# 2lambda123/CliMA-Oceananigans.jl

Hardware: AMD Instinct MI355X
Metric: cell-updates/sec per time_step!, 256^3 Nonhydrostatic WENO5 (higher is better)
Workload: dtype f64

## Files before the change

### clima-oceananigans.jl_amd/csrc/api.hip

```cpp
#include <cstdarg>

#include "internal.h"

#ifdef OCN_HOST_EMU
thread_local dim3 threadIdx, blockIdx, blockDim, gridDim;
emu_barrier g_emu_barrier;
double g_emu_shfl[4096];
std::recursive_mutex g_emu_launch_mutex;
#else
thread_local int g_ocn_dry = 0;
thread_local ocn_launch_error g_ocn_launch_err = {hipSuccess, {0}};
#endif
thread_local int g_ocn_capturing = 0, g_ocn_capture_poison = 0;

static char g_last_error[512] = {0};
static int pnhs_refresh(ocn_model* m);

void ocn_set_error(ocn_ctx* ctx, const char* fmt, ...) {
  va_list ap;
  va_start(ap, fmt);
  vsnprintf(g_last_error, sizeof(g_last_error), fmt, ap);
  va_end(ap);
  if (ctx) memcpy(ctx->err, g_last_error, sizeof(g_last_error));
}
// ... 493 lines not shown
static int pnhs_refresh(ocn_model* m) {
  if (!m->pnhs_halo_stale) return OCN_OK;
  if (int rc = halo_settle(m)) return rc;
  m->pnhs_halo_stale = false;
  Field* fs[1] = {&m->pNHS};
  return comm_halo_exchange_z(m, fs, 1);
}
static int halo_settle_others(ocn_model* m) {
  for (ocn_model* o : m->ctx->models)
    if (o != m)
      if (int rc = halo_settle_one(o)) return rc;
  return OCN_OK;
}

static int overlap_streams(ocn_ctx* c) {
  if (c->overlap_ready) return OCN_OK;
  OCN_HIP_CHECK(c, hipStreamCreate(&c->comm_stream));
  OCN_HIP_CHECK(c, hipEventCreate(&c->ev_main));
  OCN_HIP_CHECK(c, hipEventCreate(&c->ev_halo));
  OCN_HIP_CHECK(c, hipEventCreate(&c->ev_halo2));
  c->overlap_ready = true;
  return OCN_OK;
}

static int fused_substep(ocn_model* m, double dt_full, double cn, double cm, int use_m, double dt_stage, bool swap) {
  const int Hz = m->gd.Hz, Nz = m->gd.Nz;
  if (m->g->dist)
    if (int rc0 = halo_settle_others(m)) return rc0;
  if (m->halo_inflight && Nz > 2 * Hz + 2) {
    launch_fused_tend_step(m, dt_full, cn, cm, use_m, Hz, Nz - Hz);
    OCN_HIP_CHECK(m->ctx, hipStreamWaitEvent(m->ctx->stream, m->ctx->ev_halo, 0));
    m->halo_inflight = false;
    launch_fused_tend_step(m, dt_full, cn, cm, use_m, 0, Hz, Nz - Hz, Nz);
  } else {
    int rc0 = halo_settle(m);
    if (rc0) return rc0;
    launch_fused_tend_step(m, dt_full, cn, cm, use_m);
  }
  launch_tracer_steps(m, dt_full, cn, cm, use_m);
  if (m->halo2_inflight) {
    OCN_HIP_CHECK(m->ctx, hipStreamWaitEvent(m->ctx->stream, m->ctx->ev_halo2, 0));
    m->halo2_inflight = false;
  }
  int rc = OCN_OK;
  if (m->g->dist && !poisson_local_wstar(m) && (rc = fused_exchange_ws(m))) return rc;
  if (poisson_custom_xy(m)) {
    rc = poisson_run_from_predictor(m, dt_stage);
  } else {
    launch_rhs_wrap(m, dt_stage, poisson_rhs_buffer(m->solver));
    rc = poisson_run(m);
  }
  if (rc) return rc;
  if (m->g->dist && !poisson_local_phi_below(m) && (rc = fused_exchange_phi(m, poisson_rhs_buffer(m->solver)))) return rc;
  launch_project(m, dt_stage, poisson_rhs_buffer(m->solver));
  if (m->g->dist) {
    ocn_ctx* c = m->ctx;
    const size_t halo_bytes = (size_t)(3 + m->nt) * Hz * m->u.sz * sizeof(double);
    const bool want = m->knob_overlap >= 0 ? m->knob_overlap != 0 : (c->nranks > 1 && halo_bytes >= ((size_t)8 << 20));
    if (want && comm_can_overlap(c) && Nz > 2 * Hz + 2 && overlap_streams(c) == OCN_OK) {
      Field* fa[3 + OCN_MAX_TRACERS] = {&m->u, &m->v, &m->w};
      int na = 3;
      for (int t = 0; t < m->nt; ++t) fa[na++] = &m->tr[t];
      OCN_HIP_CHECK(c, hipEventRecord(c->ev_main, c->stream));
      OCN_HIP_CHECK(c, hipStreamWaitEvent(c->comm_stream, c->ev_main, 0));
      if ((rc = comm_halo_exchange_z(m, fa, na, c->comm_stream))) return rc;
      OCN_HIP_CHECK(c, hipEventRecord(c->ev_halo, c->comm_stream));
      m->halo_inflight = true;
    } else {
      Field* fs[3 + OCN_MAX_TRACERS] = {&m->u, &m->v, &m->w};
      int nf = 3;
      for (int t = 0; t < m->nt; ++t) fs[nf++] = &m->tr[t];
      if ((rc = comm_halo_exchange_z(m, fs, nf))) return rc;
    }
    m->pnhs_halo_stale = true;
  }
  if (swap)
    for (int f = 0; f < 3 + m->nt; ++f) std::swap(m->Gn[f], m->Gm[f]);
  return OCN_OK;
}

static void tendencies_and_step(ocn_model* m, double dt, double cn, double cm, int use_m) {
  if (!m->bz_fast) {
    launch_tendencies(m);
    launch_step(m, dt, cn, cm, use_m);
    return;
  }
  const bool tr3 = m->nt > 0 && fused_tracer3_ok(m);
  launch_tendencies(m, true, tr3);
  launch_fused_bz(m, dt, cn, cm, use_m);
  if (tr3) launch_tracer3(m, dt, cn, cm, use_m, true);
  else launch_step(m, dt, cn, cm, use_m, true);
  m->pred_active = true;
}

static int time_step_ab2(ocn_model* m, double dt, int force_euler) {
  bool euler = force_euler || (dt != m->previous_dt);
  double chi = euler ? -0.5 : m->d.chi;
  int rc0 = euler ? zero_Gm(m) : OCN_OK;
  if (rc0) return rc0;
  m->previous_dt = dt;
  if (m->iteration == 0 && (rc0 = update_state(m))) return rc0;
  if (m->fast_path) {
    m->gn_alias_gm = false;
    int rc = fused_substep(m, dt, 1.5 + chi, -(0.5 + chi), 1, dt, true);
    if (rc) return rc;
    m->gn_alias_gm = true;
    m->time += dt;
// ... 724 lines not shown
```

### clima-oceananigans.jl_amd/csrc/compat.h

```cpp
#pragma once

#include <cmath>
#include <cstddef>
#include <cstdint>
#include <cstdio>
#include <cstdlib>
#include <cstring>

#ifndef OCN_HOST_EMU
#include <hip/hip_runtime.h>
#include <hipfft/hipfft.h>

#define OCN_DEVFN __device__ __forceinline__

extern thread_local int g_ocn_dry;

struct ocn_launch_error {
  hipError_t err;
  char what[200];
};
extern thread_local ocn_launch_error g_ocn_launch_err;
static inline void ocn_note_error(hipError_t e, const char* what) {
  if (e == hipSuccess || g_ocn_launch_err.err != hipSuccess) return;
  g_ocn_launch_err.err = e;
  snprintf(g_ocn_launch_err.what, sizeof g_ocn_launch_err.what, "%s", what);
}
template <class K, class... A>
static inline void ocn_launch_impl(const char* what, K kern, dim3 grid, dim3 block, hipStream_t s, A... args) {
  if (g_ocn_dry) return;
  hipLaunchKernelGGL(kern, grid, block, 0, s, args...);
  ocn_note_error(hipGetLastError(), what);
}
#define ocn_launch(...) ocn_launch_impl(#__VA_ARGS__, __VA_ARGS__)
#define ocn_launch_sync(...) ocn_launch_impl(#__VA_ARGS__, __VA_ARGS__)
#define OCN_ASYNC(call) ocn_note_error((call), #call)
#define OCN_SHARED __shared__
#define OCN_SCHED_FENCE() __builtin_amdgcn_sched_barrier(0)
#define OCN_TOUCH3(a, b, c) asm volatile("" ::"v"(a), "v"(b), "v"(c))

typedef __attribute__((address_space(3))) void ocn_lds_void;
typedef const __attribute__((address_space(1))) void ocn_glb_void;
__device__ __forceinline__ void ocn_glds16(const void* src_lane, void* dst_wave_base, int ) {
  __builtin_amdgcn_global_load_lds((ocn_glb_void*)src_lane, (ocn_lds_void*)dst_wave_base, 16, 0, 0);
}
__device__ __forceinline__ double ocn_shfl_next(double x) {
  union { double d; int i[2]; } a, b;
  a.d = x;
  b.i[0] = __builtin_amdgcn_update_dpp(0, a.i[0], 0x130, 0xf, 0xf, false);
  b.i[1] = __builtin_amdgcn_update_dpp(0, a.i[1], 0x130, 0xf, 0xf, false);
  return b.d;
}
__device__ __forceinline__ double ocn_shfl_xor16(double x) {
  union { double d; int i[2]; } a, b;
  a.d = x;
  const int lane = __builtin_amdgcn_mbcnt_hi(~0u, __builtin_amdgcn_mbcnt_lo(~0u, 0u));
  const int addr = (lane ^ 16) << 2;
  b.i[0] = __builtin_amdgcn_ds_bpermute(addr, a.i[0]);
  b.i[1] = __builtin_amdgcn_ds_bpermute(addr, a.i[1]);
  return b.d;
}
#define OCN_WAVE 64
#define OCN_UNIFORM(x) __builtin_amdgcn_readfirstlane(x)

#else
#include <chrono>
#include <condition_variable>
#include <mutex>
#include <thread>
#include <vector>

struct dim3 {
  unsigned x, y, z;
  dim3(unsigned a = 1, unsigned b = 1, unsigned c = 1) : x(a), y(b), z(c) {}
};
extern thread_local dim3 threadIdx, blockIdx, blockDim, gridDim;
#define g_ocn_dry 0
extern std::recursive_mutex g_emu_launch_mutex;

#define __global__
#define __device__
#define __host__
#define __forceinline__ inline
#define __launch_bounds__(...)
#define OCN_DEVFN inline
#define OCN_SHARED static
#define OCN_SCHED_FENCE() ((void)0)
#define OCN_ASYNC(call) ((void)(call))
#define OCN_TOUCH3(a, b, c) ((void)0)

typedef int hipError_t;
enum { hipSuccess = 0, hipErrorOutOfMemory = 2 };
typedef struct emu_stream* hipStream_t;
struct emu_event { std::chrono::steady_clock::time_point t; };
typedef emu_event* hipEvent_t;
enum { hipMemcpyHostToDevice = 1, hipMemcpyDeviceToHost = 2, hipMemcpyDeviceToDevice = 3 };

static inline const char* hipGetErrorString(hipError_t) { return "host-emu error"; }
static inline hipError_t hipSetDevice(int) { return 0; }
static inline hipError_t hipGetDeviceCount(int* n) { *n = 1; return 0; }
static inline hipError_t hipStreamCreate(hipStream_t* s) { *s = nullptr; return 0; }
static inline hipError_t hipStreamDestroy(hipStream_t) { return 0; }
static inline hipError_t hipStreamSynchronize(hipStream_t) { return 0; }
static inline hipError_t hipDeviceSynchronize() { return 0; }
static inline hipError_t hipGetLastError() { return 0; }
static inline hipError_t hipMalloc(void** p, size_t n) { *p = malloc(n ? n : 1); return *p ? 0 : 2; }
static inline hipError_t hipFree(void* p) { free(p); return 0; }
static inline hipError_t hipMemcpy(void* d, const void* s, size_t n, int) { memcpy(d, s, n); return 0; }
static inline hipError_t hipMemcpyAsync(void* d, const void* s, size_t n, int, hipStream_t) { memmove(d, s, n); return 0; }
static inline hipError_t hipMemsetAsync(void* d, int v, size_t n, hipStream_t) { memset(d, v, n); return 0; }
static inline hipError_t hipMemset(void* d, int v, size_t n) { memset(d, v, n); return 0; }
static inline hipError_t hipEventCreate(hipEvent_t* e) { *e = new emu_event; return 0; }
static inline hipError_t hipEventDestroy(hipEvent_t e) { delete e; return 0; }
static inline hipError_t hipEventRecord(hipEvent_t e, hipStream_t) { e->t = std::chrono::steady_clock::now(); return 0; }
static inline hipError_t hipEventSynchronize(hipEvent_t) { return 0; }
static inline hipError_t hipStreamWaitEvent(hipStream_t, hipEvent_t, unsigned) { return 0; }
static inline hipError_t hipEventElapsedTime(float* ms, hipEvent_t a, hipEvent_t b) {
  *ms = std::chrono::duration<float, std::milli>(b->t - a->t).count();
  return 0;
}

template <class K, class... A>
static inline void ocn_launch(K kern, dim3 grid, dim3 block, hipStream_t, A... args) {
  std::lock_guard<std::recursive_mutex> lk(g_emu_launch_mutex);
  gridDim = grid;
  blockDim = block;
  for (unsigned bz = 0; bz < grid.z; ++bz)
    for (unsigned by = 0; by < grid.y; ++by)
      for (unsigned bx = 0; bx < grid.x; ++bx) {
        blockIdx = dim3(bx, by, bz);
        for (unsigned tz = 0; tz < block.z; ++tz)
          for (unsigned ty = 0; ty < block.y; ++ty)
            for (unsigned tx = 0; tx < block.x; ++tx) {
              threadIdx = dim3(tx, ty, tz);
              kern(args...);
            }
      }
}

struct emu_barrier {
  std::mutex m;
  std::condition_variable cv;
// ... 70 lines not shown
```

### clima-oceananigans.jl_amd/csrc/fused.hip

```cpp
#include "internal.h"

#define FUSED_MAX_THREADS 1024

struct FusedArgs {
  const double *u, *v, *w;
  const double *gmu, *gmv, *gmw;
  double *gnu, *gnv, *gnw;
  double *us, *vs, *ws;
  unsigned org;
  double dt, cn, cm;
  int use_m;
  int BYo;
  int ntiles;
  int ntx, BXo;
  int prio;
  double nu;
  int zlo, zhi;
  int zlo2, zhi2;
  int gran;
};

#ifndef OCN_HOST_EMU
#define OCN_SETPRIO(n) __builtin_amdgcn_s_setprio(n)
#else
// ... 469 lines not shown
          fxn[0 * BY * NW] = t11;
          fxn[1 * BY * NW] = t12;
          fxn[2 * BY * NW] = t13;
        }
      }
      if (full) {
        if (k > k0) {
          const unsigned cm1 = c - szb;
          const double rzc = ZB ? g_rdzc(g, k - 1) : g.rdz, rzfm = ZB ? g_rdzf(g, k - 1) : g.rdz;
          sto(a.gu, cm1, hu + 2.0 * ((t13 - bu) * rzc));
          sto(a.gv, cm1, hv + 2.0 * ((t23 - bv) * rzc));
          sto(a.gw, cm1, hw + 2.0 * ((t33 - bw) * rzfm));
        }
        if (!last) {
          double cu = 0, cv = 0;
          if (a.coriolis) {
            cu = a.f * (0.5 * (0.5 * (RS(1, 0, -1) + vc) + 0.5 * (RS(1, 1, -1) + RS(1, 1, 0))));
            cv = -a.f * (0.5 * (0.5 * (RS(0, -1, 0) + RS(0, -1, 1)) + 0.5 * (uc + RS(0, 0, 1))));
          }
          if (a.pH) {
            cu -= (p0 - pw) * rdx;
            cv -= (p0 - ps) * rdy;
          }
          hu = cu + 2.0 * fma(xedge ? -t11 : e0 - t11, rdx, -t12 * rdy);
          hv = cv + 2.0 * fma(xedge ? -t12 : e1 - t12, rdx, -t22 * rdy);
          hw = 2.0 * fma(xedge ? -t13 : e2 - t13, rdx, -t23 * rdy);
          bu = t13;
          bv = t23;
          bw = t33;
        }
      }
      up = uc; vp = vc; wp = wc;
      ncp = nc; nwp = nw; nsp = ns;
    }
  }
#undef RS
}

__global__ void k_rhs_wrap(GridDev g, const double* __restrict__ us, const double* __restrict__ vs,
                           const double* __restrict__ ws, double rdt, int zwrap, double* __restrict__ rhs) {
  int i, j;
  ocn_cell_ij(i, j);
  const int k = blockIdx.z;
  if (i >= g.Nx || j >= g.Ny || k >= g.Nz) return;
  const long sy = g.sy, sz = g.sz;
  const long c = i + j * sy + k * sz;
  const long ce = (i + 1 == g.Nx) ? c + 1 - g.Nx : c + 1;
  const long cn = (j + 1 == g.Ny) ? c + sy - g.Ny * sy : c + sy;
  const long ct = (zwrap && k + 1 == g.Nz) ? c + sz - g.Nz * sz : c + sz;
  double div = (us[ce] - us[c]) * g.rdx + (vs[cn] - vs[c]) * g.rdy + (ws[ct] - ws[c]) / g.dz;
  rhs[i + (long)g.Nx * (j + (long)g.Ny * k)] = div * rdt;
}

struct ProjArgs {
  const double* phi;
  const double *us, *vs, *ws;
  double *u, *v, *w, *p;
  const double* phi_below;
  double dt;
  int zwrap;
};

OCN_DEVFN void store_images(const GridDev& g, double* f, int i, int j, int k, double val, int zwrap) {
  long ox[3], oy[3], oz[3];
  int nx = 0, ny = 0, nz = 0;
  ox[nx++] = 0;
  if (i < g.Hx) ox[nx++] = g.Nx;
  if (i >= g.Nx - g.Hx) ox[nx++] = -g.Nx;
  oy[ny++] = 0;
  if (j < g.Hy) oy[ny++] = (long)g.Ny * g.sy;
  if (j >= g.Ny - g.Hy) oy[ny++] = -(long)g.Ny * g.sy;
  oz[nz++] = 0;
  if (zwrap) {
    if (k < g.Hz) oz[nz++] = (long)g.Nz * g.sz;
    if (k >= g.Nz - g.Hz) oz[nz++] = -(long)g.Nz * g.sz;
  }
  const long c = i + j * g.sy + k * g.sz;
  for (int c3 = 0; c3 < nz; ++c3)
    for (int c2 = 0; c2 < ny; ++c2)
      for (int c1 = 0; c1 < nx; ++c1) f[c + ox[c1] + oy[c2] + oz[c3]] = val;
}

__global__ void k_project(GridDev g, ProjArgs a) {
  int i, j;
  ocn_cell_ij(i, j);
  const int k = blockIdx.z;
  if (i >= g.Nx || j >= g.Ny || k >= g.Nz) return;
  const long c = i + j * g.sy + k * g.sz;
  const long Nx = g.Nx, Ny = g.Ny;
  const long pc = i + Nx * (j + Ny * k);
  const long pw_ = (i == 0) ? pc + Nx - 1 : pc - 1;
  const long ps_ = (j == 0) ? pc + Nx * (Ny - 1) : pc - Nx;
  double p0 = a.phi[pc];
  double pb;
  if (k > 0) pb = a.phi[pc - Nx * Ny];
  else if (a.zwrap) pb = a.phi[pc + Nx * Ny * (g.Nz - 1)];
  else pb = a.phi_below[i + Nx * j];
  double un = a.us[c] - (p0 - a.phi[pw_]) * g.rdx * a.dt;
  double vn = a.vs[c] - (p0 - a.phi[ps_]) * g.rdy * a.dt;
  double wn = a.ws[c] - (p0 - pb) / g.dz * a.dt;
  store_images(g, a.u, i, j, k, un, a.zwrap);
  store_images(g, a.v, i, j, k, vn, a.zwrap);
  store_images(g, a.w, i, j, k, wn, a.zwrap);
  store_images(g, a.p, i, j, k, p0, a.zwrap);
}

struct TracerArgs {
  const double *u, *v, *w, *c, *gm;
  double *gn, *cnew;
  double dt, cn, cm;
  int use_m, KZ, zwrap;
  double kappa;
};

template <int ADV>
__global__ void __launch_bounds__(256) k_tracer_step(GridDev g, TracerArgs a) {
  const int i = blockIdx.x * blockDim.x + threadIdx.x;
  const int j = blockIdx.y * blockDim.y + threadIdx.y;
  if (i >= g.Nx || j >= g.Ny) return;
  const int k0 = blockIdx.z * a.KZ;
  const int k1 = (k0 + a.KZ < g.Nz) ? k0 + a.KZ : g.Nz;
  const long sy = g.sy, sz = g.sz;
  const double rdx = g.rdx, rdy = g.rdy, rdz = 1.0 / g.dz;
  long c = i + j * sy + (long)k0 * sz;
  double zc[6];
#pragma unroll
  for (int q = 0; q < 6; ++q) zc[q] = a.c[c + (q - 3) * sz];
  auto fz = [&](long p) {
    const double wt = a.w[p];
    const bool pos = wt > 0.0;
    return wt * recon5<ADV>(pos ? zc[0] : zc[5], pos ? zc[1] : zc[4], pos ? zc[2] : zc[3], pos ? zc[3] : zc[2],
                            pos ? zc[4] : zc[1], pos) - a.kappa * (zc[3] - zc[2]) * rdz;
  };
  double fb = fz(c);
  for (int k = k0; k < k1; ++k, c += sz) {
// ... 171 lines not shown
          const unsigned cm1 = c - szb;
          const double rzc = ZB ? g_rdzc(g, k - 1) : g.rdz;
          const double G = rest - (own_h + (fb - own_b) * rzc);
          sto(a.gn, cm1, G);
          const double inc = a.use_m ? a.dt * (a.cn * G + a.cm * gmv) : a.dt * a.cn * G;
          const double val = zc[2] + inc;
          if (IMG) store_images(g, (double*)((char*)a.cnew + a.org), i, j, k - 1, val, a.zwrap);
          else sto(a.cnew, cm1, val);
        }
        if (!last) {
          own_h = (fxx[nid_e] - fxx[tid]) * rdx + (fxy[nid_n] - fxy[tid]) * rdy;
          own_b = fb;
        }
      }
      if (!last) {
#pragma unroll
        for (int q = 0; q < 5; ++q) zc[q] = zc[q + 1];
        zc[5] = ldo(a.c, c + 3 * szb);
      }
    }
  }
#undef CS
#undef KS
}

static const char* tiled_blocker(const ocn_model* m) {
  const ocn_grid* g = m->g;
  const int adv = m->d.advection;
  if (adv != ADV_WENO_Z && adv != ADV_WENO_JS && adv != ADV_U5) return "the advection scheme is not an upwind-biased 5th-order one";
  for (int d = 0; d < 3; ++d)
    if (g->topo[d] != OCN_FLAT && (g->H[d] < 3 || g->N[d] < 2 * g->H[d])) return "a direction has fewer than 6 cells";
  if (m->u.n * sizeof(double) >= (1ull << 31) || m->w.n * sizeof(double) >= (1ull << 31))
    return "parent arrays of 2 GiB or more exceed the tiled kernels' 32-bit byte offsets";
  return nullptr;
}

bool fused_available(const ocn_model* m) {
  const ocn_grid* g = m->g;
  if (g->topo[0] != OCN_PERIODIC || g->topo[1] != OCN_PERIODIC || g->topo[2] != OCN_PERIODIC) return false;
  if (!g->z_regular) return false;
  if (m->d.closure == OCN_CLOSURE_AMD || m->d.coriolis_fplane || m->d.buoyancy != OCN_BUOYANCY_NONE) return false;
  if (tiled_blocker(m)) return false;
  if (getenv("OCNHIP_NO_FUSED")) return false;
  return true;
}

bool rest4_ok(const ocn_model* m);
void fused_describe(const ocn_model* m, char* buf, size_t n) {
  const char* why = tiled_blocker(m);
  if (m->fast_path) {
    const size_t halo_bytes = (size_t)(3 + m->nt) * m->gd.Hz * m->u.sz * sizeof(double);
    const bool ov = m->g->dist && m->gd.Nz > 2 * m->gd.Hz + 2 &&
                    (m->knob_overlap >= 0 ? m->knob_overlap != 0 : (m->ctx->nranks > 1 && halo_bytes >= ((size_t)8 << 20)));
    snprintf(buf, n, "all-in-one periodic path: k_tend4 + fused Poisson passes + k_project%s",
             !m->g->dist ? "" : ov ? "; z-slabs, halo planes travel under the next interior tendency launch"
                                   : "; z-slabs, halo exchange on the model's stream");
  }
  else if (m->bz_fast) snprintf(buf, n, "tiled advection + update (k_tend4, REST) on top of the %s other terms",
                                rest4_ok(m) ? "tiled kernel's (k_rest4)" : "general kernels'");
  else if (why) snprintf(buf, n, "general kernels: %s", why);
  else if (m->g->topo[0] == OCN_FLAT || m->g->topo[1] == OCN_FLAT) snprintf(buf, n, "general kernels: Flat x / y slices are outside the tiled kernels");
  else snprintf(buf, n, "general kernels (tiled path disabled or not applicable to this topology / decomposition)");
}

static int fused_cu_count(const ocn_model* m) {
  static int ncu = 0;
  if (!ncu) {
#ifndef OCN_HOST_EMU
    hipDeviceProp_t prop;
    ncu = (hipGetDeviceProperties(&prop, m->ctx->device) == hipSuccess) ? prop.multiProcessorCount : 256;
#else
    ncu = 8;
#endif
  }
  return ncu;
}

struct FusedShape {
  int bx, by;
  bool wide, small;
  int dma;
  dim3 blk, grd;
};

void fused_read_knobs(ocn_model* m) {
  auto env = [](const char* n, int def) { const char* e = getenv(n); return e ? atoi(e) : def; };
  m->knob_fused_xt = env("OCNHIP_FUSED_XT", 0);
  m->knob_no_dma = env("OCNHIP_NO_LDS_DMA", 0);
  m->knob_no_tracer3 = env("OCNHIP_NO_TRACER3", 0);
  m->knob_xfft_team = env("OCNHIP_XFFT_TEAM", 0);
  m->knob_overlap = env("OCNHIP_OVERLAP", -1);
  m->knob_overlap_cus = env("OCNHIP_OVERLAP_CUS", 16);
  m->knob_graph = env("OCNHIP_NO_GRAPH", 0) ? 0 : 1;
  { const char* e = getenv("OCNHIP_PRIO"); m->knob_prio = e ? (int)strtol(e, nullptr, 0) : 0x20FF; }
}

static FusedShape fused_shape(const ocn_model* m, FusedArgs& a) {
  const GridDev& gd = m->gd;
  FusedShape f;
  f.small = m->knob_fused_xt == 1 && gd.Nx <= 57 * 4;
#ifdef OCN_HOST_EMU
  if (gd.xb && gd.Nx <= 57 * 4) f.small = true;
#endif
  f.wide = gd.Nx > 256 || f.small || gd.xb;
  f.bx = f.small ? 64 : f.wide ? 192 : gd.Nx <= 64 ? 64 : gd.Nx <= 128 ? 128 : 256;
  f.by = f.small ? 4 : f.wide ? 5 : f.bx == 256 ? 4 : 8;
#ifdef OCN_HOST_EMU
  if ((f.small && gd.Nx <= 36) || (!f.wide && gd.Nx <= 16)) {
    f.bx = 16;
    f.by = 4;
  }
#endif
  a.BYo = f.by - 1;
  a.ntiles = (gd.Ny + f.by - 2) / (f.by - 1);
  a.ntx = 1;
  a.BXo = 0;
  if (f.wide) {
    const int cap = (f.bx - 7) & ~1;
    a.ntx = (gd.Nx + cap - 1) / cap;
    if (f.small && a.ntx < 2) a.ntx = 2;
    a.BXo = (gd.Nx + a.ntx - 1) / a.ntx;
    a.BXo += a.BXo & 1;
    a.ntx = (gd.Nx + a.BXo - 1) / a.BXo;
    a.ntiles *= a.ntx;
  }
  int nseg = fused_cu_count(m);
  const long total = (long)a.ntiles * ((a.zhi - a.zlo) + (a.zhi2 - a.zlo2));
  a.gran = 1;
  if (a.zhi2 > a.zlo2) {
    a.gran = a.zhi - a.zlo;
    const long runs = total / a.gran;
    if (nseg > runs) nseg = (int)runs;
  } else {
    if (a.zhi - a.zlo < gd.Nz && nseg > 4 * m->knob_overlap_cus) nseg -= m->knob_overlap_cus;
    if (nseg > total / 4) nseg = (int)(total / 4 > 8 ? total / 4 : 8);
    nseg = ((nseg + 7) / 8) * 8;
  }
#ifdef OCN_HOST_EMU
  nseg = total >= 3 ? 3 : 1;
#endif
  f.blk = dim3(f.bx, f.by, 1);
  f.grd = dim3(nseg, 1, 1);
  f.dma = (m->knob_no_dma != 1 && gd.Hx == 3 && gd.Nx % 2 == 0 && gd.sy % 2 == 0 && gd.sz % 2 == 0) ? 1 : 0;
// ... 281 lines not shown
```

### clima-oceananigans.jl_amd/csrc/internal.h

```cpp
#pragma once
#include <map>
#include <string>
#include <vector>

#include "../../include/ocnhip.h"
#include "compat.h"
#include "stencils.h"

#define OCN_NF (3 + OCN_MAX_TRACERS)

struct ProfPhase {
  std::vector<std::pair<hipEvent_t, hipEvent_t>> ev;
  double total_ms = 0;
  int64_t count = 0;
};

struct ocn_ctx {
  int device = 0;
  hipStream_t stream = nullptr;
  char err[512] = {0};
  bool profiling = false;
  std::map<std::string, ProfPhase> prof;
  std::string prof_only;
  int rank = 0, nranks = 1;
// ... 41 lines not shown
};

struct Field {
  double* d = nullptr;
  int T[3] = {0, 0, 0};
  int P[3] = {0, 0, 0};
  int off[3] = {0, 0, 0};
  int loc[3] = {0, 0, 0};
  size_t n = 0;
  BCdev bc[6];
  bool present = false;
  double* interior() const;
  long sy = 0, sz = 0;
  int Hx = 0, Hy = 0, Hz = 0;
};

struct PoissonSolver;

struct ocn_model {
  ocn_grid* g;
  ocn_ctx* ctx;
  ocn_model_desc d;
  GridDev gd;
  int nt;
  Field u, v, w, pHY, pNHS;
  Field tr[OCN_MAX_TRACERS], Gn[OCN_NF], Gm[OCN_NF];
  Field nu_e, kappa_e[OCN_MAX_TRACERS];
  Field us, vs, ws;
  Field trs[OCN_MAX_TRACERS];
  PoissonSolver* solver = nullptr;
  std::vector<double*> owned;
  double time = 0, previous_dt = INFINITY;
  int64_t iteration = 0;
  int stage = 1;
  double* d_red = nullptr;
  int fast_path = 0;
  int bz_fast = 0;
  double* amd_tab = nullptr;
  double* phi_below = nullptr;
  double *ypack_s = nullptr, *ypack_r = nullptr;
  size_t ypack_n = 0;
  bool gn_alias_gm = false;
  bool pred_active = false;
  ocn_grid* own_grid = nullptr;
  int knob_fused_xt = 0, knob_no_dma = 0, knob_no_tracer3 = 0, knob_prio = 0x20FF;
  struct StepGraph { uint64_t key; int seen; void* exec; std::vector<uint64_t> words; };
  std::vector<StepGraph> graphs;
  int knob_overlap_cus = 16;
  int knob_overlap = -1;
  bool halo_inflight = false, halo2_inflight = false;
  bool pnhs_halo_stale = false;
  int knob_xfft_team = 0;
  int knob_graph = 1;
  bool graph_off = false;
  int64_t graph_replays = 0;
};
extern thread_local int g_ocn_capturing, g_ocn_capture_poison;
inline Field& pred_u(ocn_model* m) { return m->pred_active ? m->us : m->u; }
inline Field& pred_v(ocn_model* m) { return m->pred_active ? m->vs : m->v; }
inline Field& pred_w(ocn_model* m) { return m->pred_active ? m->ws : m->w; }

Field* model_field(ocn_model* m, int id);

struct FieldPtrs {
  double* p[OCN_NF + 2];
  int Tx[OCN_NF + 2], Ty[OCN_NF + 2], Tz[OCN_NF + 2];
  int n;
};
void launch_fill_periodic(ocn_model* m, const FieldPtrs& f, int dim);
void launch_fill_flat(ocn_model* m, const FieldPtrs& f, int dim);
bool launch_fill_periodic_xy(ocn_model* m, const FieldPtrs& f);
void launch_fill_bounded(ocn_model* m, Field** fs, int n, int dim);
void launch_tendencies(ocn_model* m, bool skip_momentum_advection = false, bool skip_tracer_advection = false);
void launch_step(ocn_model* m, double dt, double cn, double cm, int use_m, bool tracers_only = false);
void launch_store(ocn_model* m);
void launch_rhs(ocn_model* m, double dt, double* rhs, int mult_dz);
void launch_pcorrect(ocn_model* m, double dt);
void launch_hydrostatic(ocn_model* m);
void launch_copy_to_field(ocn_model* m, const double* src, Field& f);
void launch_maxdiv(ocn_model* m, double* out_dev);
void launch_amd(ocn_model* m);
int amd_build_table(ocn_model* m);

void fused_read_knobs(ocn_model* m);
void fused_describe(const ocn_model* m, char* buf, size_t n);
bool fused_available(const ocn_model* m);
bool fused_bz_available(const ocn_model* m);
void launch_fused_bz(ocn_model* m, double dt, double cn, double cm, int use_m);
bool launch_rest4(ocn_model* m);
bool fused_tracer3_ok(const ocn_model* m);
bool tracer_rest_shell(const ocn_model* m);
void launch_tracer3(ocn_model* m, double dt, double cn, double cm, int use_m, bool rest);
void launch_fused_tend_step(ocn_model* m, double dt, double cn, double cm, int use_m, int zlo = 0, int zhi = -1, int zlo2 = 0, int zhi2 = 0);
void launch_rhs_wrap(ocn_model* m, double dt, double* rhs);
void launch_project(ocn_model* m, double dt, const double* phi);
void launch_tracer_steps(ocn_model* m, double dt, double cn, double cm, int use_m);
int fused_exchange_ws(ocn_model* m);
int fused_exchange_phi(ocn_model* m, const double* phi);
int poisson_run(ocn_model* m);

PoissonSolver* poisson_create(ocn_model* m);
void poisson_destroy(PoissonSolver* s);
int poisson_solve(ocn_model* m, double dt);
int poisson_solve_rhs(ocn_model* m, const double* rhs_dev, double* phi_dev);
double* poisson_rhs_buffer(PoissonSolver* s);

void* zsolve_create(ocn_ctx* ctx, const std::vector<double>& lx_half, const std::vector<double>& ly_local);
void zsolve_destroy(void* z);
void zsolve_run(ocn_ctx* ctx, void* z, void* spec, int Nz, const double* lz, double norm, long zero_col);
void yfft_run(ocn_ctx* ctx, void* z, void* spec, int Nxh, int Ny, int Nz, int inverse);
void xfft_rhs_run(ocn_model* m, void* z, void* spec, double dt, int extra_plane = 0);
bool poisson_local_wstar(const ocn_model* m);
bool fft_size_ok(int n);
bool zsolve_size_ok(int n);
bool poisson_custom_xy(const ocn_model* m);
int poisson_run_from_predictor(ocn_model* m, double dt);

void* zslab_create(ocn_ctx* ctx, const std::vector<double>& lx_half, const std::vector<double>& ly, int n, int R, int rank);
void zslab_destroy(void* z);
int zslab_run(ocn_ctx* ctx, void* z, void* spec, double dz2, double scale, const void* below = nullptr, void* phi_below = nullptr);
bool poisson_local_phi_below(const ocn_model* m);
const double* poisson_phi_below(const ocn_model* m);

int comm_exchange(ocn_ctx* c, const std::vector<CommOp>& sends, const std::vector<CommOp>& recvs, hipStream_t st = nullptr);
int comm_halo_exchange_z(ocn_model* m, Field** fs, int n, hipStream_t st = nullptr);
bool comm_can_overlap(const ocn_ctx* c);
int halo_settle(ocn_model* m);
int comm_halo_exchange_y(ocn_model* m, Field** fs, int n);
int comm_alltoall(ocn_ctx* c, const void* send, void* recv, size_t block_bytes);
void comm_destroy(ocn_ctx* c);

struct ProfScope {
  ocn_ctx* c;
  hipEvent_t a = nullptr, b = nullptr;
  const char* name;
  ProfScope(ocn_ctx* ctx, const char* nm);
  ~ProfScope();
};
```

### clima-oceananigans.jl_amd/csrc/poisson.hip

```cpp
#include "internal.h"
#ifndef OCN_HOST_EMU
#define dry_hipfftExecD2Z(...) (g_ocn_dry ? HIPFFT_SUCCESS : hipfftExecD2Z(__VA_ARGS__))
#define dry_hipfftExecZ2D(...) (g_ocn_dry ? HIPFFT_SUCCESS : hipfftExecZ2D(__VA_ARGS__))
#define dry_hipfftExecZ2Z(...) (g_ocn_dry ? HIPFFT_SUCCESS : hipfftExecZ2Z(__VA_ARGS__))
#endif


#ifndef OCN_HOST_EMU
#include <rocblas/rocblas.h>
#endif
#include <complex>
typedef std::complex<double> cplx;

struct double2_ {
  double x, y;
};

struct PoissonSolver {
  int kind;
  int Nx, Ny, Nz, Nxh;
  int R = 1, rank = 0, Nzg = 0, Nyl = 0;
  double2_ *ta = nullptr, *tb = nullptr;
  void* zs = nullptr;
  void* zsl = nullptr;
// ... 1009 lines not shown
  }
  return OCN_OK;
}

int poisson_run(ocn_model* m) { return run_solver(m); }

bool poisson_custom_xy(const ocn_model* m) { return m->solver && m->solver->cxy; }
bool poisson_local_wstar(const ocn_model* m) { return m->solver && m->solver->bplane != nullptr; }
bool poisson_local_phi_below(const ocn_model* m) { return m->solver && m->solver->bplane != nullptr && m->solver->local_phi; }
const double* poisson_phi_below(const ocn_model* m) { return m->solver->rhs + (size_t)m->solver->Nx * m->solver->Ny * m->solver->Nz; }

#ifdef OCN_HOST_EMU
static void emu_xinv(PoissonSolver* s, const double2_* spec = nullptr, double* out = nullptr, size_t nlines = 0) {
  const int Nx = s->Nx, Nxh = s->Nxh;
  const size_t lines = nlines ? nlines : (size_t)s->Ny * s->Nz;
  if (!spec) spec = s->spec;
  if (!out) out = s->rhs;
  std::vector<cplx> full(Nx);
  for (size_t L = 0; L < lines; ++L) {
    for (int i = 0; i < Nx; ++i) {
      double2_ q = spec[(i < Nxh ? i : Nx - i) + Nxh * L];
      full[i] = cplx(q.x, i < Nxh ? q.y : -q.y);
    }
    for (int n = 0; n < Nx; ++n) {
      cplx acc = 0;
      for (int i = 0; i < Nx; ++i) {
        double ang = 2.0 * M_PI * ((long)i * n % Nx) / Nx;
        acc += full[i] * cplx(cos(ang), sin(ang));
      }
      out[n + Nx * L] = acc.real();
    }
  }
}
#endif

int poisson_run_from_predictor(ocn_model* m, double dt) {
  PoissonSolver* s = m->solver;
  const int xp = s->bplane ? 1 : 0, ip = (s->bplane && s->local_phi) ? 1 : 0;
  {
    ProfScope ps(m->ctx, "fft_forward");
    xfft_rhs_run(m, s->tw, s->spec, dt, xp);
    yfft_run(m->ctx, s->tw, s->spec, s->Nxh, s->Ny, s->Nz + xp, 0);
  }
  if (s->zs) {
    ProfScope ps(m->ctx, "spectral_solve");
    zsolve_run(m->ctx, s->zs, s->spec, s->Nz, s->lz, 1.0 / ((double)s->Nx * s->Ny * s->Nz), 0);
  } else {
    int rc = zslab_run(m->ctx, s->zsl, s->spec, s->dz2, 1.0 / ((double)s->Nx * s->Ny), s->bplane, ip ? s->bplane : nullptr);
    if (rc) return rc;
  }
  {
    ProfScope ps(m->ctx, "fft_backward");
    yfft_run(m->ctx, s->tw, s->spec, s->Nxh, s->Ny, s->Nz + ip, 1);
#ifndef OCN_HOST_EMU
    if (dry_hipfftExecZ2D(s->xinv, (hipfftDoubleComplex*)s->spec, s->rhs) != HIPFFT_SUCCESS) {
      ocn_set_error(m->ctx, "hipfftExecZ2D (x inverse) failed");
      return OCN_EHIP;
    }
#else
    emu_xinv(s, s->spec, s->rhs, (size_t)s->Ny * (s->Nz + ip));
#endif
  }
  return OCN_OK;
}

static int poisson_run_from_predictor_bz(ocn_model* m, double dt) {
  PoissonSolver* s = m->solver;
  {
    ProfScope ps(m->ctx, "fft_forward");
    xfft_rhs_run(m, s->tw, s->spec, dt);
    yfft_run(m->ctx, s->tw, s->spec, s->Nxh, s->Ny, s->Nz, 0);
  }
  {
    ProfScope ps(m->ctx, "spectral_solve");
    tridiag_run(m, s, s->Nxh, s->Ny, s->lx, s->ly, 1.0 / ((double)s->Nx * s->Ny), s->spec, 1);
  }
  {
    ProfScope ps(m->ctx, "fft_backward");
    yfft_run(m->ctx, s->tw, s->spec, s->Nxh, s->Ny, s->Nz, 1);
#ifndef OCN_HOST_EMU
    if (dry_hipfftExecZ2D(s->xinv, (hipfftDoubleComplex*)s->spec, s->rhs) != HIPFFT_SUCCESS) {
      ocn_set_error(m->ctx, "hipfftExecZ2D (x inverse) failed");
      return OCN_EHIP;
    }
#else
    emu_xinv(s);
#endif
  }
  return OCN_OK;
}

int poisson_solve(ocn_model* m, double dt) {
  PoissonSolver* s = m->solver;
  int rc;
  if (s->cxy_bz) rc = poisson_run_from_predictor_bz(m, dt);
  else {
    launch_rhs(m, dt, s->rhs, m->g->topo[2] == OCN_BOUNDED ? 1 : 0);
    rc = run_solver(m);
  }
  if (rc) return rc;
  ProfScope ps(m->ctx, "copy_pressure");
  launch_copy_to_field(m, s->rhs, m->pNHS);
  return OCN_OK;
}

__global__ void k_mult_dz(GridDev g, double* __restrict__ r) {
  int i, j;
  ocn_cell_ij(i, j);
  const int k = blockIdx.z;
  if (i >= g.Nx || j >= g.Ny || k >= g.Nz) return;
  r[i + (size_t)g.Nx * (j + (size_t)g.Ny * k)] *= g_dzc(g, k);
}

int poisson_solve_rhs(ocn_model* m, const double* rhs_dev, double* phi_dev) {
  PoissonSolver* s = m->solver;
  size_t nr = (size_t)s->Nx * s->Ny * s->Nz;
  OCN_ASYNC(hipMemcpyAsync(s->rhs, rhs_dev, nr * sizeof(double), hipMemcpyDeviceToDevice, m->ctx->stream));
// ... 10 lines not shown
```

### clima-oceananigans.jl_amd/csrc/zfft.hip

```cpp
#include "internal.h"

struct cd {
  double x, y;
};
OCN_DEVFN cd cadd(cd a, cd b) { return {a.x + b.x, a.y + b.y}; }
OCN_DEVFN cd csub(cd a, cd b) { return {a.x - b.x, a.y - b.y}; }
OCN_DEVFN cd cmul(cd a, cd b) { return {a.x * b.x - a.y * b.y, a.x * b.y + a.y * b.x}; }
template <int S> OCN_DEVFN cd mul_mi(cd a) { return S > 0 ? cd{a.y, -a.x} : cd{-a.y, a.x}; }

template <int S> OCN_DEVFN void dft4(cd& a, cd& b, cd& c, cd& d) {
  cd s0 = cadd(a, c), s1 = csub(a, c), s2 = cadd(b, d), s3 = mul_mi<S>(csub(b, d));
  a = cadd(s0, s2);
  c = csub(s0, s2);
  b = cadd(s1, s3);
  d = csub(s1, s3);
}

template <int S> OCN_DEVFN void dft16(cd* v) {
#pragma unroll
  for (int a = 0; a < 4; ++a) dft4<S>(v[a], v[a + 4], v[a + 8], v[a + 12]);
  const double C1 = 0.92387953251128673848, S1 = 0.38268343236508978178, R = 0.70710678118654752440;
  auto tw = [&](cd z, double c, double s) { return cd{z.x * c + S * z.y * s, z.y * c - S * z.x * s}; };
  v[1 + 4] = tw(v[1 + 4], C1, S1);
  v[1 + 8] = tw(v[1 + 8], R, R);
// ... 428 lines not shown
      const int l2 = e / N, i = e - l2 * N;
      int j = j0 + l2, k = k0;
      while (j >= g.Ny) { j -= g.Ny; ++k; }
      double d = 0.0;
      if (extra && k == g.Nz) d = ws[j * sy + i] * rdz * rdt;
      else if (k < g.Nz) {
        const long row = j * sy + k * sz;
        const long rown = ((j + 1 == g.Ny) ? 0 : j + 1) * sy + k * sz;
        const long rowt = (zwrap && k + 1 == g.Nz) ? j * sy : j * sy + (k + 1) * sz;
        const int ie = (i + 1 == g.Nx) ? 0 : i + 1;
        if (g.zb) {
          const double dzc = g_dzc(g, k);
          d = ((us[row + ie] - us[row + i]) * g.rdx + (vs[rown + i] - vs[row + i]) * g.rdy + (ws[rowt + i] - ws[row + i]) / dzc) * rdt * dzc;
        } else
        d = ((us[row + ie] - us[row + i]) * g.rdx + (vs[rown + i] - vs[row + i]) * g.rdy + (ws[rowt + i] - ws[row + i]) * rdz) * rdt;
      }
      sm[l2 * LP + i] = d;
    }
    __syncthreads();
#pragma unroll
    for (int n1 = 0; n1 < 16; ++n1) v[n1] = {sm[ln * LP + pos_in<N>(r, c, n1)], 0.0};
    __syncthreads();
  } else {
    const int k = ok ? (int)(L / g.Ny) : 0, j = ok ? (int)(L - (long)k * g.Ny) : 0;
    const long row = j * sy + k * sz;
    const long rown = ((j + 1 == g.Ny) ? 0 : j + 1) * sy + k * sz;
    const long rowt = (zwrap && k + 1 == g.Nz) ? j * sy : j * sy + (k + 1) * sz;
#pragma unroll
    for (int n1 = 0; n1 < 16; ++n1) {
      const int i = pos_in<N>(r, c, n1);
      const int ie = (i + 1 == g.Nx) ? 0 : i + 1;
      double d = 0.0;
      if (ok && extra && k == g.Nz) d = ws[j * sy + i] * rdz * rdt;
      else if (ok && g.zb) {
        const double dzc = g_dzc(g, k);
        d = ((us[row + ie] - us[row + i]) * g.rdx + (vs[rown + i] - vs[row + i]) * g.rdy + (ws[rowt + i] - ws[row + i]) / dzc) * rdt * dzc;
      } else if (ok) d = ((us[row + ie] - us[row + i]) * g.rdx + (vs[rown + i] - vs[row + i]) * g.rdy + (ws[rowt + i] - ws[row + i]) * rdz) * rdt;
      v[n1] = {d, 0.0};
    }
  }
  fft_fwd<N, 1, true>(sm, v, r, c, tw);
  if (ok) {
    cd* out = spec + L * (N / 2 + 1);
#pragma unroll
    for (int q = 0; q < 16; ++q) {
      const int kmin = N == 128 ? 8 * (q >> 3) + 16 * (q & 7) : N == 256 ? 16 * q : 32 * q;
      if (kmin > N / 2) continue;
      const int kx = pos_out<N>(r, c, q);
      if (kx <= N / 2) out[kx] = v[q];
    }
  }
}

struct ZSolve {
  cd* twmr = nullptr;
  int twmr_n = 0;
  cd* tw = nullptr;
  double* lxy = nullptr;
  long ncol = 0;
};

bool fft_size_ok(int n) { return n == 128 || n == 256 || n == 512; }
bool zsolve_size_ok(int n) { return fft_size_ok(n) || n == 320 || n == 384; }

void* zsolve_create(ocn_ctx* ctx, const std::vector<double>& lx_half, const std::vector<double>& ly_local) {
  ZSolve* z = new ZSolve;
  const size_t Nxh = lx_half.size(), Ny = ly_local.size();
  z->ncol = (long)(Nxh * Ny);
  std::vector<double> lxy(Nxh * Ny);
  for (size_t j = 0; j < Ny; ++j)
    for (size_t i = 0; i < Nxh; ++i) lxy[i + Nxh * j] = lx_half[i] + ly_local[j];
  std::vector<cd> tw(512);
  for (int m = 0; m < 512; ++m) tw[m] = {cos(2.0 * M_PI * m / 512.0), -sin(2.0 * M_PI * m / 512.0)};
  if (hipMalloc((void**)&z->tw, sizeof(cd) * 512) != hipSuccess ||
      hipMalloc((void**)&z->lxy, sizeof(double) * lxy.size()) != hipSuccess) {
    ocn_set_error(ctx, "zsolve: allocation failed");
    delete z;
    return nullptr;
  }
  hipMemcpy(z->tw, tw.data(), sizeof(cd) * 512, hipMemcpyHostToDevice);
  hipMemcpy(z->lxy, lxy.data(), sizeof(double) * lxy.size(), hipMemcpyHostToDevice);
  return z;
}

void zsolve_destroy(void* p) {
  ZSolve* z = (ZSolve*)p;
  if (!z) return;
  hipFree(z->twmr);
  hipFree(z->tw);
  hipFree(z->lxy);
  delete z;
}

#define FFT_BY_N(N, CALL128, CALL256, CALL512) \
  switch (N) { case 128: CALL128; break; case 256: CALL256; break; default: CALL512; break; }

void yfft_run(ocn_ctx* ctx, void* p, void* spec, int Nxh, int Ny, int Nz, int inverse) {
  ZSolve* z = (ZSolve*)p;
  const int C = 256 / (Ny / 16);
  const int nfull = Nxh / C, left = Nxh - C * nfull;
  const long nblk = (long)nfull * Nz + ((long)left * Nz + C - 1) / C;
  dim3 b(256, 1, 1), g((unsigned)nblk, 1, 1);
  cd* a = (cd*)spec;
  const cd* tw = (const cd*)z->tw;
  hipStream_t s = ctx->stream;
  if (inverse) {
    FFT_BY_N(Ny, ocn_launch_sync(k_yfft<128, -1>, g, b, s, a, Nxh, Nz, tw), ocn_launch_sync(k_yfft<256, -1>, g, b, s, a, Nxh, Nz, tw),
             ocn_launch_sync(k_yfft<512, -1>, g, b, s, a, Nxh, Nz, tw))
  } else {
    FFT_BY_N(Ny, ocn_launch_sync(k_yfft<128, 1>, g, b, s, a, Nxh, Nz, tw), ocn_launch_sync(k_yfft<256, 1>, g, b, s, a, Nxh, Nz, tw),
             ocn_launch_sync(k_yfft<512, 1>, g, b, s, a, Nxh, Nz, tw))
  }
}

void xfft_rhs_run(ocn_model* m, void* p, void* spec, double dt, int extra_plane) {
  ZSolve* z = (ZSolve*)p;
  const GridDev& g = m->gd;
  const long nlines = (long)g.Ny * (g.Nz + (extra_plane ? 1 : 0));
  const int ex = extra_plane;
  const int C = 256 / (g.Nx / 16);
  dim3 b(256, 1, 1), gr((unsigned)((nlines + C - 1) / C), 1, 1);
  const double* us = (m->fast_path ? m->us : pred_u(m)).interior();
  const double* vs = (m->fast_path ? m->vs : pred_v(m)).interior();
  const double* ws = (m->fast_path ? m->ws : pred_w(m)).interior();
  const int zw = (m->g->dist || m->g->topo[2] != OCN_PERIODIC) ? 0 : 1;
  hipStream_t s = m->ctx->stream;
  cd* sp = (cd*)spec;
  const cd* tw = (const cd*)z->tw;
  if (m->knob_xfft_team) {
    FFT_BY_N(g.Nx, ocn_launch_sync(k_xfft_rhs<128, false>, gr, b, s, g, us, vs, ws, 1.0 / dt, zw, sp, tw, ex),
             ocn_launch_sync(k_xfft_rhs<256, false>, gr, b, s, g, us, vs, ws, 1.0 / dt, zw, sp, tw, ex),
             ocn_launch_sync(k_xfft_rhs<512, false>, gr, b, s, g, us, vs, ws, 1.0 / dt, zw, sp, tw, ex))
  } else {
    FFT_BY_N(g.Nx, ocn_launch_sync(k_xfft_rhs<128, true>, gr, b, s, g, us, vs, ws, 1.0 / dt, zw, sp, tw, ex),
             ocn_launch_sync(k_xfft_rhs<256, true>, gr, b, s, g, us, vs, ws, 1.0 / dt, zw, sp, tw, ex),
             ocn_launch_sync(k_xfft_rhs<512, true>, gr, b, s, g, us, vs, ws, 1.0 / dt, zw, sp, tw, ex))
  }
}

void zsolve_run(ocn_ctx* ctx, void* p, void* spec, int Nz, const double* lz, double norm, long zero_col) {
  ZSolve* z = (ZSolve*)p;
  if (Nz == 320 || Nz == 384) {
    if (z->twmr_n != Nz) {
      std::vector<cd> t(Nz);
      for (int m = 0; m < Nz; ++m) t[m] = {cos(2.0 * M_PI * m / Nz), -sin(2.0 * M_PI * m / Nz)};
      hipStreamSynchronize(ctx->stream);
      hipFree(z->twmr);
      z->twmr = nullptr;
      z->twmr_n = 0;
      if (hipMalloc((void**)&z->twmr, sizeof(cd) * Nz) != hipSuccess) {
        ocn_set_error(ctx, "zsolve: allocation failed");
        return;
      }
      hipMemcpy(z->twmr, t.data(), sizeof(cd) * Nz, hipMemcpyHostToDevice);
      z->twmr_n = Nz;
    }
    dim3 g((unsigned)((z->ncol + 15) / 16), 1, 1);
    cd* a = (cd*)spec;
    if (Nz == 320)
      ocn_launch_sync(k_zsolve_mr<20>, g, dim3(320, 1, 1), ctx->stream, a, z->ncol, (const double*)z->lxy, lz, (const cd*)z->twmr, norm, zero_col);
    else
      ocn_launch_sync(k_zsolve_mr<24>, g, dim3(384, 1, 1), ctx->stream, a, z->ncol, (const double*)z->lxy, lz, (const cd*)z->twmr, norm, zero_col);
    return;
  }
  const int C = 256 / (Nz / 16);
  dim3 b(256, 1, 1), g((unsigned)((z->ncol + C - 1) / C), 1, 1);
  cd* a = (cd*)spec;
  const cd* tw = (const cd*)z->tw;
  hipStream_t s = ctx->stream;
  FFT_BY_N(Nz, ocn_launch_sync(k_zsolve<128>, g, b, s, a, z->ncol, (const double*)z->lxy, lz, tw, norm, zero_col),
           ocn_launch_sync(k_zsolve<256>, g, b, s, a, z->ncol, (const double*)z->lxy, lz, tw, norm, zero_col),
           ocn_launch_sync(k_zsolve<512>, g, b, s, a, z->ncol, (const double*)z->lxy, lz, tw, norm, zero_col))
}
```

Baseline: 15.50 billion.

## Fuse inverse x-FFT into pressure projection kernel

Skips the hipFFT Z2D inverse x transform and adds a kernel that does the inverse real FFT per z-level in LDS, then immediately applies the pressure-gradient projection to u, v, w and stores p. The goal is to avoid writing the real-space pressure field to global memory and reading it back in a separate projection kernel. The kernel keeps two z-levels in LDS so it can form the vertical gradient, splits the domain into y-tiles and z-segments, and recomputes some overlapping rows and levels. It applies only on the non-distributed fast path and can be turned off with an environment variable.

```diff
diff --git a/clima-oceananigans.jl_amd/csrc/api.hip b/clima-oceananigans.jl_amd/csrc/api.hip
--- a/clima-oceananigans.jl_amd/csrc/api.hip
+++ b/clima-oceananigans.jl_amd/csrc/api.hip
@@ -569,7 +569,8 @@
   }
   if (rc) return rc;
   if (m->g->dist && !poisson_local_phi_below(m) && (rc = fused_exchange_phi(m, poisson_rhs_buffer(m->solver)))) return rc;
-  launch_project(m, dt_stage, poisson_rhs_buffer(m->solver));
+  if (poisson_xinv_fused(m)) poisson_xinv_project(m, dt_stage);
+  else launch_project(m, dt_stage, poisson_rhs_buffer(m->solver));
   if (m->g->dist) {
     ocn_ctx* c = m->ctx;
     const size_t halo_bytes = (size_t)(3 + m->nt) * Hz * m->u.sz * sizeof(double);
diff --git a/clima-oceananigans.jl_amd/csrc/compat.h b/clima-oceananigans.jl_amd/csrc/compat.h
--- a/clima-oceananigans.jl_amd/csrc/compat.h
+++ b/clima-oceananigans.jl_amd/csrc/compat.h
@@ -37,6 +37,8 @@
 #define OCN_SHARED __shared__
 #define OCN_SCHED_FENCE() __builtin_amdgcn_sched_barrier(0)
 #define OCN_TOUCH3(a, b, c) asm volatile("" ::"v"(a), "v"(b), "v"(c))
+#define OCN_OPAQUE_SPTR(p) asm volatile("" : "+s"(p))
+#define OCN_OPAQUE_V(x) asm volatile("" : "+v"(x))
 
 typedef __attribute__((address_space(3))) void ocn_lds_void;
 typedef const __attribute__((address_space(1))) void ocn_glb_void;
@@ -87,6 +89,8 @@
 #define OCN_SCHED_FENCE() ((void)0)
 #define OCN_ASYNC(call) ((void)(call))
 #define OCN_TOUCH3(a, b, c) ((void)0)
+#define OCN_OPAQUE_SPTR(p) ((void)0)
+#define OCN_OPAQUE_V(x) ((void)0)
 
 typedef int hipError_t;
 enum { hipSuccess = 0, hipErrorOutOfMemory = 2 };
diff --git a/clima-oceananigans.jl_amd/csrc/fused.hip b/clima-oceananigans.jl_amd/csrc/fused.hip
--- a/clima-oceananigans.jl_amd/csrc/fused.hip
+++ b/clima-oceananigans.jl_amd/csrc/fused.hip
@@ -545,35 +545,6 @@
   rhs[i + (long)g.Nx * (j + (long)g.Ny * k)] = div * rdt;
 }
 
-struct ProjArgs {
-  const double* phi;
-  const double *us, *vs, *ws;
-  double *u, *v, *w, *p;
-  const double* phi_below;
-  double dt;
-  int zwrap;
-};
-
-OCN_DEVFN void store_images(const GridDev& g, double* f, int i, int j, int k, double val, int zwrap) {
-  long ox[3], oy[3], oz[3];
-  int nx = 0, ny = 0, nz = 0;
-  ox[nx++] = 0;
-  if (i < g.Hx) ox[nx++] = g.Nx;
-  if (i >= g.Nx - g.Hx) ox[nx++] = -g.Nx;
-  oy[ny++] = 0;
-  if (j < g.Hy) oy[ny++] = (long)g.Ny * g.sy;
-  if (j >= g.Ny - g.Hy) oy[ny++] = -(long)g.Ny * g.sy;
-  oz[nz++] = 0;
-  if (zwrap) {
-    if (k < g.Hz) oz[nz++] = (long)g.Nz * g.sz;
-    if (k >= g.Nz - g.Hz) oz[nz++] = -(long)g.Nz * g.sz;
-  }
-  const long c = i + j * g.sy + k * g.sz;
-  for (int c3 = 0; c3 < nz; ++c3)
-    for (int c2 = 0; c2 < ny; ++c2)
-      for (int c1 = 0; c1 < nx; ++c1) f[c + ox[c1] + oy[c2] + oz[c3]] = val;
-}
-
 __global__ void k_project(GridDev g, ProjArgs a) {
   int i, j;
   ocn_cell_ij(i, j);
@@ -851,7 +822,8 @@
     const size_t halo_bytes = (size_t)(3 + m->nt) * m->gd.Hz * m->u.sz * sizeof(double);
     const bool ov = m->g->dist && m->gd.Nz > 2 * m->gd.Hz + 2 &&
                     (m->knob_overlap >= 0 ? m->knob_overlap != 0 : (m->ctx->nranks > 1 && halo_bytes >= ((size_t)8 << 20)));
-    snprintf(buf, n, "all-in-one periodic path: k_tend4 + fused Poisson passes + k_project%s",
+    snprintf(buf, n, "all-in-one periodic path: k_tend4 + fused Poisson passes + %s%s",
+             poisson_xinv_fused(m) ? "k_xinv_project (inverse x transform inside the projection)" : "k_project",
              !m->g->dist ? "" : ov ? "; z-slabs, halo planes travel under the next interior tendency launch"
                                    : "; z-slabs, halo exchange on the model's stream");
   }
@@ -862,7 +834,7 @@
   else snprintf(buf, n, "general kernels (tiled path disabled or not applicable to this topology / decomposition)");
 }
 
-static int fused_cu_count(const ocn_model* m) {
+int fused_cu_count(const ocn_model* m) {
   static int ncu = 0;
   if (!ncu) {
 #ifndef OCN_HOST_EMU
@@ -888,6 +860,7 @@
   m->knob_no_dma = env("OCNHIP_NO_LDS_DMA", 0);
   m->knob_no_tracer3 = env("OCNHIP_NO_TRACER3", 0);
   m->knob_xfft_team = env("OCNHIP_XFFT_TEAM", 0);
+  m->knob_no_xinv_project = env("OCNHIP_NO_XINV_PROJECT", 0);
   m->knob_overlap = env("OCNHIP_OVERLAP", -1);
   m->knob_overlap_cus = env("OCNHIP_OVERLAP_CUS", 16);
   m->knob_graph = env("OCNHIP_NO_GRAPH", 0) ? 0 : 1;
diff --git a/clima-oceananigans.jl_amd/csrc/internal.h b/clima-oceananigans.jl_amd/csrc/internal.h
--- a/clima-oceananigans.jl_amd/csrc/internal.h
+++ b/clima-oceananigans.jl_amd/csrc/internal.h
@@ -117,6 +117,7 @@
   bool pnhs_halo_stale = false;
   int knob_xfft_team = 0;
   int knob_graph = 1;
+  int knob_no_xinv_project = 0;
   bool graph_off = false;
   int64_t graph_replays = 0;
 };
@@ -159,6 +160,34 @@
 void launch_fused_tend_step(ocn_model* m, double dt, double cn, double cm, int use_m, int zlo = 0, int zhi = -1, int zlo2 = 0, int zhi2 = 0);
 void launch_rhs_wrap(ocn_model* m, double dt, double* rhs);
 void launch_project(ocn_model* m, double dt, const double* phi);
+int fused_cu_count(const ocn_model* m);
+struct ProjArgs {
+  const double* phi;
+  const double *us, *vs, *ws;
+  double *u, *v, *w, *p;
+  const double* phi_below;
+  double dt;
+  int zwrap;
+};
+OCN_DEVFN void store_images(const GridDev& g, double* f, int i, int j, int k, double val, int zwrap) {
+  long ox[3], oy[3], oz[3];
+  int nx = 0, ny = 0, nz = 0;
+  ox[nx++] = 0;
+  if (i < g.Hx) ox[nx++] = g.Nx;
+  if (i >= g.Nx - g.Hx) ox[nx++] = -g.Nx;
+  oy[ny++] = 0;
+  if (j < g.Hy) oy[ny++] = (long)g.Ny * g.sy;
+  if (j >= g.Ny - g.Hy) oy[ny++] = -(long)g.Ny * g.sy;
+  oz[nz++] = 0;
+  if (zwrap) {
+    if (k < g.Hz) oz[nz++] = (long)g.Nz * g.sz;
+    if (k >= g.Nz - g.Hz) oz[nz++] = -(long)g.Nz * g.sz;
+  }
+  const long c = i + j * g.sy + k * g.sz;
+  for (int c3 = 0; c3 < nz; ++c3)
+    for (int c2 = 0; c2 < ny; ++c2)
+      for (int c1 = 0; c1 < nx; ++c1) f[c + ox[c1] + oy[c2] + oz[c3]] = val;
+}
 void launch_tracer_steps(ocn_model* m, double dt, double cn, double cm, int use_m);
 int fused_exchange_ws(ocn_model* m);
 int fused_exchange_phi(ocn_model* m, const double* phi);
@@ -180,6 +209,9 @@
 bool zsolve_size_ok(int n);
 bool poisson_custom_xy(const ocn_model* m);
 int poisson_run_from_predictor(ocn_model* m, double dt);
+bool poisson_xinv_fused(const ocn_model* m);
+void poisson_xinv_project(ocn_model* m, double dt);
+void xinv_project_run(ocn_model* m, void* z, const void* spec, double dt);
 
 void* zslab_create(ocn_ctx* ctx, const std::vector<double>& lx_half, const std::vector<double>& ly, int n, int R, int rank);
 void zslab_destroy(void* z);
diff --git a/clima-oceananigans.jl_amd/csrc/poisson.hip b/clima-oceananigans.jl_amd/csrc/poisson.hip
--- a/clima-oceananigans.jl_amd/csrc/poisson.hip
+++ b/clima-oceananigans.jl_amd/csrc/poisson.hip
@@ -1085,6 +1085,7 @@
   {
     ProfScope ps(m->ctx, "fft_backward");
     yfft_run(m->ctx, s->tw, s->spec, s->Nxh, s->Ny, s->Nz + ip, 1);
+    if (poisson_xinv_fused(m)) return OCN_OK;
 #ifndef OCN_HOST_EMU
     if (dry_hipfftExecZ2D(s->xinv, (hipfftDoubleComplex*)s->spec, s->rhs) != HIPFFT_SUCCESS) {
       ocn_set_error(m->ctx, "hipfftExecZ2D (x inverse) failed");
@@ -1096,6 +1097,11 @@
   }
   return OCN_OK;
 }
+
+bool poisson_xinv_fused(const ocn_model* m) {
+  return m->fast_path && m->solver && m->solver->cxy && !m->g->dist && !m->knob_no_xinv_project;
+}
+void poisson_xinv_project(ocn_model* m, double dt) { xinv_project_run(m, m->solver->tw, m->solver->spec, dt); }
 
 static int poisson_run_from_predictor_bz(ocn_model* m, double dt) {
   PoissonSolver* s = m->solver;
diff --git a/clima-oceananigans.jl_amd/csrc/zfft.hip b/clima-oceananigans.jl_amd/csrc/zfft.hip
--- a/clima-oceananigans.jl_amd/csrc/zfft.hip
+++ b/clima-oceananigans.jl_amd/csrc/zfft.hip
@@ -504,6 +504,138 @@
   }
 }
 
+template <int N> struct XipGeo {
+  static constexpr int C = FftGeo<N>::C;
+  static constexpr int R = C - 1;
+  static constexpr int NXH = N / 2 + 1;
+  static constexpr int LP = N + 16;
+  static constexpr int NPRE = (C * NXH + 255) / 256;
+  static constexpr int PER = (R * N + 255) / 256;
+};
+
+template <int N>
+__global__ void __launch_bounds__(256, 2) k_xinv_project(GridDev g, ProjArgs a, const cd* __restrict__ spec, const cd* __restrict__ tw,
+                                                      int nseg, int ntiles) {
+  typedef XipGeo<N> X;
+  static_assert(2 * X::C * X::NXH <= SMN && X::C * X::LP <= SMN, "spectrum rows and real rows must fit the transform's LDS buffer");
+  static_assert(2 * SMN * sizeof(double) <= OCN_LDS_BYTES / 2, "two workgroups per CU");
+  OCN_SHARED double buf[2][SMN];
+  constexpr int M = FftGeo<N>::M;
+  const int t = threadIdx.x;
+  const int rr = t % M, ln = t / M;
+  const int r = N == 512 ? rr & 15 : rr;
+  const int c = N == 512 ? ln + 8 * (rr >> 4) : ln;
+  long b = blockIdx.x;
+  const long nb = gridDim.x;
+  if (nb % 8 == 0) b = (b % 8) * (nb / 8) + b / 8;
+  const int tile = (int)(b % ntiles), sg = (int)(b / ntiles);
+  const int j0 = tile * X::R;
+  const int k0 = (int)((long)sg * g.Nz / nseg), nlev = (int)((long)(sg + 1) * g.Nz / nseg) - k0;
+  const int Ny = g.Ny;
+
+  cd pre[X::NPRE];
+  auto fetch = [&](int k) {
+#pragma unroll
+    for (int m = 0; m < X::NPRE; ++m) {
+      const int e = t + 256 * m;
+      const int l = e / X::NXH, kx = e - l * X::NXH;
+      int j = j0 - 1 + l;
+      if (j < 0) j += Ny;
+      const bool ok = l < X::C && j < Ny;
+      pre[m] = ok ? spec[kx + X::NXH * ((long)j + (long)Ny * k)] : cd{0, 0};
+    }
+  };
+  constexpr bool AHEAD = N != 512;
+  constexpr int CH = AHEAD ? (X::PER + 1) / 2 : 4;
+  int tl = t;
+  auto cell = [&](int m, int& l, int& i, int& j) {
+    const int e = tl + 256 * m;
+    l = 1 + e / N;
+    i = e & (N - 1);
+    j = j0 + l - 1;
+    return l < X::C && j < Ny;
+  };
+  struct Pred { double us[CH], vs[CH], ws[CH]; };
+  auto load_pred = [&](Pred& f, int k, int m0) {
+#pragma unroll
+    for (int q = 0; q < CH; ++q) {
+      int l, i, j;
+      const bool ok = cell(m0 + q, l, i, j);
+      const long cc = i + j * g.sy + k * g.sz;
+      f.us[q] = ok ? a.us[cc] : 0.0;
+      f.vs[q] = ok ? a.vs[cc] : 0.0;
+      f.ws[q] = ok ? a.ws[cc] : 0.0;
+    }
+  };
+  auto project = [&](const Pred& f, int k, int m0, const double* cur, const double* prv) {
+#pragma unroll
+    for (int q = 0; q < CH; ++q) {
+      int l, i, j;
+      if (!cell(m0 + q, l, i, j)) continue;
+      const double p0 = cur[l * X::LP + i];
+      const double pw = cur[l * X::LP + (i == 0 ? N - 1 : i - 1)];
+      const double ps = cur[(l - 1) * X::LP + i];
+      const double pb = prv[l * X::LP + i];
+      double un = f.us[q] - (p0 - pw) * g.rdx * a.dt;
+      double vn = f.vs[q] - (p0 - ps) * g.rdy * a.dt;
+      double wn = f.ws[q] - (p0 - pb) / g.dz * a.dt;
+      store_images(g, a.u, i, j, k, un, 1);
+      store_images(g, a.v, i, j, k, vn, 1);
+      store_images(g, a.w, i, j, k, wn, 1);
+      store_images(g, a.p, i, j, k, p0, 1);
+      OCN_SCHED_FENCE();
+    }
+  };
+  Pred fa, fb;
+  if (AHEAD) fetch(k0 == 0 ? g.Nz - 1 : k0 - 1);
+  for (int s = -1; s < nlev; ++s) {
+    const int k = k0 + s;
+    double* cur = buf[(s + 1) & 1];
+    const double* prv = buf[s & 1];
+    cd* stg = (cd*)cur;
+    if (!AHEAD) fetch(s < 0 && k0 == 0 ? g.Nz - 1 : k);
+    OCN_OPAQUE_V(tl);
+    __syncthreads();
+#pragma unroll
+    for (int m = 0; m < X::NPRE; ++m) {
+      const int e = t + 256 * m;
+      if (e < X::C * X::NXH) stg[e] = pre[m];
+    }
+    if (AHEAD && s >= 0) load_pred(fa, k, 0);
+    __syncthreads();
+    cd v[16];
+#pragma unroll
+    for (int n1 = 0; n1 < 16; ++n1) {
+      const int kk = pos_in<N>(r, c, n1);
+      cd z = stg[ln * X::NXH + (kk <= N / 2 ? kk : N - kk)];
+      if (kk > N / 2) z.y = -z.y;
+      v[n1] = z;
+    }
+    __syncthreads();
+    const cd* twl = tw;
+    OCN_OPAQUE_SPTR(twl);
+    fft_fwd<N, -1, N != 512>(cur, v, r, c, twl);
+    __syncthreads();
+#pragma unroll
+    for (int q = 0; q < 16; ++q) cur[ln * X::LP + pos_out<N>(r, c, q)] = v[q].x;
+    if (AHEAD && s + 1 < nlev) fetch(k + 1);
+    __syncthreads();
+    if (s < 0) continue;
+    OCN_OPAQUE_V(tl);
+    if (AHEAD) {
+      load_pred(fb, k, CH);
+      project(fa, k, 0, cur, prv);
+      project(fb, k, CH, cur, prv);
+    } else {
+#pragma unroll 1
+      for (int m0 = 0; m0 < X::PER; m0 += CH) {
+        load_pred(fa, k, m0);
+        project(fa, k, m0, cur, prv);
+      }
+    }
+  }
+}
+
 struct ZSolve {
   cd* twmr = nullptr;
   int twmr_n = 0;
@@ -590,6 +722,36 @@
   }
 }
 
+int xinv_project_segments(int Nx, int Nz) {
+  const int C = 256 / (Nx / 16);
+  int len = 1;
+  while (100 * (len + 1 + C) > 15 * C * (len + 1)) ++len;
+  return Nz / len > 0 ? Nz / len : 1;
+}
+int xinv_project_tiles(int Nx, int Ny) { return (Ny + 256 / (Nx / 16) - 2) / (256 / (Nx / 16) - 1); }
+
+void xinv_project_run(ocn_model* m, void* p, const void* spec, double dt) {
+  ProfScope ps(m->ctx, "pcorrect");
+  ZSolve* z = (ZSolve*)p;
+  const GridDev& g = m->gd;
+  ProjArgs a;
+  a.phi = nullptr;
+  a.phi_below = nullptr;
+  a.us = m->us.interior(); a.vs = m->vs.interior(); a.ws = m->ws.interior();
+  a.u = m->u.interior(); a.v = m->v.interior(); a.w = m->w.interior(); a.p = m->pNHS.interior();
+  a.dt = dt;
+  a.zwrap = 1;
+  const int ntiles = xinv_project_tiles(g.Nx, g.Ny);
+  const int nseg = xinv_project_segments(g.Nx, g.Nz);
+  dim3 b(256, 1, 1), gr((unsigned)(ntiles * nseg), 1, 1);
+  const cd* sp = (const cd*)spec;
+  const cd* tw = (const cd*)z->tw;
+  hipStream_t s = m->ctx->stream;
+  FFT_BY_N(g.Nx, ocn_launch_sync(k_xinv_project<128>, gr, b, s, g, a, sp, tw, nseg, ntiles),
+           ocn_launch_sync(k_xinv_project<256>, gr, b, s, g, a, sp, tw, nseg, ntiles),
+           ocn_launch_sync(k_xinv_project<512>, gr, b, s, g, a, sp, tw, nseg, ntiles))
+}
+
 void zsolve_run(ocn_ctx* ctx, void* p, void* spec, int Nz, const double* lz, double norm, long zero_col) {
   ZSolve* z = (ZSolve*)p;
   if (Nz == 320 || Nz == 384) {
```

Measured after the change: 13.54 billion. 0.873x the previous value.
